# nikizadehgfdl/ocean_model_grid_generator

Measured on AMD Instinct MI355X. Metric: supergrid cells/sec (coords+metrics), 1/8° tripolar at 1/2/4/8 MI355X, higher is better.
Workload: dtype f64

## Files before the change

include/ogg_hip.h:

```cpp
#ifndef OGG_HIP_H
#define OGG_HIP_H

#ifdef __cplusplus
extern "C" {
#endif

#define OGG_OK 0
#define OGG_EORDER 1
#define OGG_ESHAPE 2
#define OGG_EHIP 3
#define OGG_ENOMEM 4
#define OGG_EARG 5

#define OGG_DP_ARC_LITERAL 0
#define OGG_DP_ARC_CHORD 1

#define OGG_SYM_DEFAULT 0
#define OGG_SYM_MIRROR 1
#define OGG_SYM_NONE 2

const char* ogg_last_error(void);
const char* ogg_version(void);
long ogg_abi_sizeof(int which);
int ogg_device_count(int* count);
// ... 177 lines not shown
    long workspace_bytes;
    int symmetry;
} ogg_dpole_band;
long ogg_dpole_band_workspace_bytes(int order, long Ni, long n_pt_rows);
int ogg_symmetry_coverage(int which, int order, long n, double lon0, double lon_dp, int symmetry, int* cell_writes, int* col_writes,
                          long* evaluated);
int ogg_supergrid_pass_dev(int n_latlon, const ogg_latlon_band* latlon, long ni1, double lon0, double lenlon, double Re, int metrics,
                           const ogg_bipolar_band* cap, const ogg_dpole_band* south_cap, void** events5, double* alg_bytes4,
                           void* stream);
int ogg_supergrid_pass_plan_dev(int n_latlon, const ogg_latlon_band* latlon, long ni1, double lon0, double lenlon, double Re, int metrics,
                                const ogg_bipolar_band* cap, const ogg_dpole_band* south_cap, void** plan_out);
int ogg_supergrid_pass_run_dev(void* plan, void** events5, double* alg_bytes4, void* stream);
int ogg_supergrid_pass_plan_destroy(void* plan);
long ogg_supergrid_pass_plan_slots(const void* plan);
long ogg_supergrid_pass_plan_carried_runs(const void* plan);
int ogg_supergrid_pass_plan_flags_dev(const void* plan, int* flags, void* stream);

int ogg_fill_dev(long n, double value, double* out, void* stream);
int ogg_bswap64_dev(long n, const void* src, void* dst, void* stream);
int ogg_libm_check_dev(int which, long n, const double* x, const double* y, unsigned long long* n_diff, void* stream);
int ogg_metrics_sums_dev(long n_dx_rows, long n_cell_rows, long ni, const double* dx, const double* dy, const double* area,
                         long col_a, long col_b, int want_first_row, int want_last_row, double* out5, void* stream);
#define OGG_QUALITY_DEGENERATE_M 1.0e-3
#define OGG_QUALITY_N_BINS 7
#define OGG_QUALITY_BIN_EDGES_DEG {1.0e-6, 1.0e-3, 0.1, 1.0, 5.0, 20.0}
enum {
    OGG_Q_DX_MIN = 0, OGG_Q_DX_MAX, OGG_Q_DY_MIN, OGG_Q_DY_MAX, OGG_Q_AREA_MIN, OGG_Q_AREA_MAX, OGG_Q_ASPECT_MAX, OGG_Q_DELTA_MAX,
    OGG_Q_RX_MAX, OGG_Q_RY_MAX, OGG_Q_RY_NEXT_MAX, OGG_Q_SEAM_MAX, OGG_Q_N_EXTREMA
};
enum {
// ... 268 lines not shown
```

ocean_model_grid_generator_amd/_lib.py:

```python
import ctypes
import os

import numpy as np

_HERE = os.path.dirname(os.path.abspath(__file__))
LIB_PATH = os.environ.get("OGG_LIB_PATH") or os.path.join(_HERE, "csrc", "libogg_hip.so")

OGG_OK, OGG_EORDER, OGG_ESHAPE, OGG_EHIP, OGG_ENOMEM, OGG_EARG = 0, 1, 2, 3, 4, 5
DP_ARC_LITERAL, DP_ARC_CHORD = 0, 1
SYM_DEFAULT, SYM_MIRROR, SYM_NONE = 0, 1, 2

c_long, c_int, c_double, c_void_p, c_longlong = ctypes.c_long, ctypes.c_int, ctypes.c_double, ctypes.c_void_p, ctypes.c_longlong
_dp = ctypes.POINTER(ctypes.c_double)
_llp = ctypes.POINTER(ctypes.c_longlong)

class LatlonBand(ctypes.Structure):
    _fields_ = [("axis_kind", c_int), ("a0", c_double), ("len", c_double), ("denom", c_double), ("y0", c_longlong),
                ("lat1d", c_void_p), ("k0", c_long), ("n_pt_rows", c_long), ("n_cell_rows", c_long), ("x", c_void_p),
                ("y", c_void_p), ("dx", c_void_p), ("dy", c_void_p), ("area", c_void_p), ("angle", c_void_p)]


class BipolarBand(ctypes.Structure):
    _fields_ = [("Ni", c_long), ("Nj", c_long), ("lat0_bp", c_double), ("lon_bp", c_double), ("rp", c_double), ("Re", c_double),
                ("order", c_int), ("symmetry", c_int), ("j0", c_long), ("n_pt_rows", c_long), ("n_cell_rows", c_long), ("x", c_void_p),
# ... 305 lines not shown
    "ogg_event_create": [ctypes.POINTER(c_void_p)],
    "ogg_event_destroy": [c_void_p],
    "ogg_event_record": [c_void_p, c_void_p],
    "ogg_event_elapsed_ms": [c_void_p, c_void_p, ctypes.POINTER(ctypes.c_float)],
    "ogg_stream_synchronize": [c_void_p],
}
STRING_GETTERS = ("ogg_last_error", "ogg_version")
LONG_GETTERS = {"ogg_abi_sizeof": [c_int],
                "ogg_bipolar_quad_workspace_bytes": [c_int, c_long, c_long],
                "ogg_displaced_pole_quad_workspace_bytes": [c_int, c_long, c_long],
                "ogg_displaced_pole_grid_workspace_bytes": [c_long, c_long],
                "ogg_dpole_band_workspace_bytes": [c_int, c_long, c_long],
                "ogg_latlon_rows_workspace_bytes": [c_int, ctypes.POINTER(LatlonBand), c_long],
                "ogg_supergrid_pass_plan_slots": [c_void_p],
                "ogg_supergrid_pass_plan_carried_runs": [c_void_p],
                "ogg_grid_quality_result_bytes": [],
                "ogg_grid_quality_workspace_bytes": [c_long, c_long],
                "ogg_topog_record_bytes": [],
                "ogg_topog_band_out_rows": [ctypes.POINTER(TopogBand)],
                "ogg_topog_workspace_bytes": [],
                "ogg_xgrid_struct_bytes": [c_int],
                "ogg_xgrid_band_first_row": [ctypes.POINTER(XgridBand)],
                "ogg_xgrid_band_out_rows": [ctypes.POINTER(XgridBand)],
                "ogg_xgrid_band_next_rows": [ctypes.POINTER(XgridBand)],
                "ogg_xgrid_workspace_bytes": [ctypes.POINTER(XgridBand), ctypes.POINTER(XgridAtm)],
                "ogg_mask_struct_bytes": [c_int],
                "ogg_mask_workspace_bytes": [ctypes.POINTER(MaskParams)],
                "ogg_remap_struct_bytes": [c_int],
                "ogg_remap_workspace_bytes": [ctypes.POINTER(RemapParams)],
                "ogg_runoff_struct_bytes": [c_int],
# ... 23 lines not shown
        try:
            import torch
        except ImportError:
            pass
    lib = ctypes.CDLL(LIB_PATH)
    for name, argtypes in SIGNATURES.items():
        if os.environ.get("OGG_LIB_PATH") and not hasattr(lib, name):
            continue
        fn = getattr(lib, name)
        fn.argtypes = argtypes
        fn.restype = c_int
    for name in STRING_GETTERS:
        getattr(lib, name).restype = ctypes.c_char_p
        getattr(lib, name).argtypes = []
    for name, argtypes in LONG_GETTERS.items():
        getattr(lib, name).restype = c_long
        getattr(lib, name).argtypes = argtypes
    _lib = lib
    return lib


def check(code):
    if code == OGG_OK:
        return
    text = load().ogg_last_error().decode("utf-8", "replace")
    if code in (OGG_EORDER, OGG_ESHAPE):
        raise Exception(text)
    raise OggHipError(code, "libogg_hip: %s" % text)


# ... 31 lines not shown
```

ocean_model_grid_generator_amd/csrc/ogg_bipolar_dev.h:

```cpp
#pragma once
#include <cstdlib>

#include "ogg_common.h"
#include "ogg_math.h"

namespace {

using namespace ogg;

struct BpRow {
    double sphig;
    double beta2_inv;
    double N_inv;
};
struct BpCol {
    double sinla;
    double alpha2;
};

OGG_DEV BpRow bp_row(double phig_in, double rp) {
    BpRow r;
    const double phig = 90 - div_pi180(2 * atan(tan(0.5 * (90 - phig_in) * kPi180) / rp));
    const double pr = phig * kPi180;
    r.sphig = sin(pr);
// ... 335 lines not shown
    m.rows_per_wg = (int)rpw;
    return dim3((unsigned)gx, (unsigned)((m.nrows + rpw - 1) / rpw));
}

constexpr double BP_GUARD_K_DEFAULT = 4000.0;

struct QuadParams {
    long nx, ny;
    double lat0_bp, lon_bp, rp, Re;
    long j0;
    long top_out_row;
    double guard_k;
    unsigned* ll_claims;
    unsigned* fix_count;
    unsigned* fix_list;
    const BpRow* row_tab;
    const BpCol* col_tab;
    double* dxq;
    double* dyq;
    double* daq;
    const double* top_src;
    QuadNodes q;
    double sx, sy, rp2p, rp2m, rp2x4, cdx, guard_kk;
};

constexpr int QS_CELLS = 63;
constexpr int QS_WAVES = 4;
constexpr int QS_WG_CELLS = QS_CELLS * QS_WAVES;

struct QuadCols {
// ... 115 lines not shown
    if (lane % M == 0 && cell < CW && c0 + cell < p.nx) p.dxq[p.top_out_row * p.nx + c0 + cell] = quad_average_1d<N>(y) * p.Re;
}

template <int N>
OGG_DEV void bipolar_tables_body(const QuadParams& p, long bx) {
    constexpr int M = N - 1;
    const long nb_tab = tables_only_blocks<N>(p);
    if (bx >= nb_tab) {
        bipolar_top_row_body<N>(p, (bx - nb_tab) * 4 + (threadIdx.x >> 6));
        return;
    }
    BpRow* row_tab = const_cast<BpRow*>(p.row_tab);
    BpCol* col_tab = const_cast<BpCol*>(p.col_tab);
    const long k = bx * blockDim.x + threadIdx.x;
    const long n_rows = M * p.ny + 2, n_cols = M * p.nx + 1;
    if (k == 0) *p.fix_count = 0u;
    for (long w = k; w < QUAD_LL_CLAIM_WORDS; w += nb_tab * blockDim.x) p.ll_claims[w] = 0u;
    if (k < n_rows) {
        double jv;
        if (k == M * p.ny)
            jv = (double)p.ny - 0.001;
        else if (k == M * p.ny + 1)
            jv = lattice_node(p.q, 0, p.ny);
        else
            jv = lattice_node(p.q, (int)(k % M), k / M);
        const double latg = p.lat0_bp + (jv * (90 - p.lat0_bp)) / (double)p.ny;
        row_tab[k] = bp_row(latg, p.rp);
    } else if (k < n_rows + n_cols) {
        const long u = k - n_rows;
        const double iv = lattice_node(p.q, (int)(u % M), u / M);
        const double lon = p.lon_bp + (iv * 360.0) / (double)p.nx;
// ... 80 lines not shown
                if (ii == 0) o.dy0 = dy;
            } else {
                const double xy = Xn * Yn;
                o.pr[ii] = (xy * rsqrt_c3(fmax(xy * (q2 * q2), tiny))) * cpr;
            }
        }
        o.guarded = 0;
        if (MODE == QM_GUARD) o.guarded = g_any | wave_next(g_first);
    }
    if (FAITHFUL) o.guarded = 0;
    if (FAITHFUL || want_dx) o.dx[M] = wave_next(o.dx[0]);
    o.pr[M] = wave_next(o.pr[0]);
}

template <int N, int MODE>
OGG_DEV void bipolar_quad_body(const QuadParams& p, const QuadRange& rg, QuadOutLds& out, long wgx, long by) {
    constexpr int M = N - 1;
    constexpr bool FAITHFUL = (MODE == QM_LITERAL);
    const int lane = threadIdx.x & 63, wave = threadIdx.x >> 6;
    const QuadLane ql = quad_lane(rg.cols, wgx, wave, lane);
    if (ql.nv == 0) return;
    const bool active = ql.active;
    const long ci = ql.ci, c0 = ql.c0;
    const int nv = ql.nv;
    const long n_cols_tab = M * p.nx + 1;
    BpCol col[M];
#pragma unroll
    for (int ii = 0; ii < M; ++ii) {
        long u = M * ci + ii;
        if (u > n_cols_tab - 1) u = n_cols_tab - 1;
        col[ii] = p.col_tab[u];
    }
    const bool cell_lane = ql.cell_lane, closing = ql.closing;
    const bool img_col = (MODE == QM_FAST) && ql.img_col;
    const long h2 = p.nx / 2;
    const QuadStores qs = quad_stores(rg.cols, ql, p.nx, MODE == QM_FAST);
// ... 49 lines not shown
                da = d * d * (Y(0, 0) + Y(0, 2) + Y(2, 0) + Y(2, 2) + 4.0 * (Y(0, 1) + Y(1, 0) + Y(1, 2) + Y(2, 1) + 4.0 * Y(1, 1)));
            } else {
                const double d = (N == 4) ? (1.0 / 12.0) : (1.0 / 180.0);
                da = d * d * ysum;
            }
            da = da * p.Re * p.Re;
        }
        const long out_r = c - p.j0;
        double* __restrict__ rdx = p.dxq + out_r * p.nx;
        double* __restrict__ rdy = p.dyq + out_r * (p.nx + 1);
        double* __restrict__ rda = p.daq + out_r * p.nx;
        if (closing) {
            rdy[ci] = dyq;
            if (img_col) rdy[h2 - ci] = dyq, rdy[h2 + ci] = dyq, rdy[p.nx - ci] = dyq;
        }
        if (cell_lane && MODE == QM_GUARD && guarded) p.fix_list[atomicAdd(p.fix_count, 1u)] = (unsigned)(out_r * p.nx + ci);
        double(*buf)[QS_WG_CELLS] = out.v[(c - r0) & 1];
        if (lane < QS_CELLS) buf[0][slot] = dxq, buf[1][slot] = dyq, buf[2][slot] = da;
        __syncthreads();
        wg_store_aligned(rdx + c0, nv, buf[0], 0, 1, wave, lane);
        wg_store_aligned(rdy + c0, nv, buf[1], 0, 1, wave, lane);
        wg_store_aligned(rda + c0, nv, buf[2], 0, 1, wave, lane);
        const int last = nv - 1;
        if (qs.n_ic > 0) {
            wg_store_aligned(rdx + qs.cell_up, qs.n_ic, buf[0], qs.k0, 1, wave, lane);
            wg_store_aligned(rda + qs.cell_up, qs.n_ic, buf[2], qs.k0, 1, wave, lane);
            wg_store_aligned(rdx + qs.cell_dn2, qs.n_ic, buf[0], last, -1, wave, lane);
            wg_store_aligned(rda + qs.cell_dn2, qs.n_ic, buf[2], last, -1, wave, lane);
            wg_store_aligned(rdx + qs.cell_dn4, qs.n_ic, buf[0], last, -1, wave, lane);
            wg_store_aligned(rda + qs.cell_dn4, qs.n_ic, buf[2], last, -1, wave, lane);
        }
        if (qs.n_ip > 0) {
            wg_store_aligned(rdy + qs.col_up, qs.n_ip, buf[1], qs.k1, 1, wave, lane);
            wg_store_aligned(rdy + qs.col_dn2, qs.n_ip, buf[1], last, -1, wave, lane);
            wg_store_aligned(rdy + qs.col_dn4, qs.n_ip, buf[1], last, -1, wave, lane);
        }
    }
}

template <int N, int MODE>
__global__ __launch_bounds__(64 * QS_WAVES) void bipolar_quad_kernel(QuadParams p, QuadRange rg) {
    __shared__ QuadOutLds out;
    bipolar_quad_body<N, MODE>(p, rg, out, blockIdx.x, blockIdx.y);
}

template <int N>
__global__ __launch_bounds__(64) void bipolar_quad_tail_kernel(QuadParams p) {
    constexpr int M = N - 1;
    __shared__ double sdx[64], sdy[64];
    const unsigned bid = blockIdx.x, nblk = gridDim.x;
    const unsigned count = *p.fix_count;
    const int lane = threadIdx.x, half = lane >> 5, q = lane & 31;
    if (p.top_src && p.top_out_row >= 0)
        for (long i = (long)bid * 64 + lane; i < p.nx; i += (long)nblk * 64) p.dxq[p.top_out_row * p.nx + i] = p.top_src[i];
    const int jj = (q < N * N) ? q / N : 0, ii = (q < N * N) ? q % N : 0;
    for (unsigned k0 = bid * 2; k0 < count; k0 += nblk * 2) {
        const unsigned k = k0 + half;
        const bool have = k < count;
        const unsigned lin = have ? p.fix_list[k] : 0u;
        const long out_r = lin / p.nx, ci = lin % p.nx;
        const long cj = p.j0 + out_r;
        double dx = 0.0, dy = 0.0;
        if (have && q < N * N) {
            const BpRow r = p.row_tab[M * cj + jj];
            const BpCol c = p.col_tab[M * ci + ii];
            double phis, rden, h_i, h_j;
            bp_point(r, c, p.rp, phis, h_i, h_j, rden);
            dx = h_i * 2 * kPi / (double)p.nx;
            dy = h_j * (90 - p.lat0_bp) * kPi180 / (double)p.ny;
        }
        __syncthreads();
        sdx[lane] = dx;
        sdy[lane] = dy;
        __syncthreads();
        if (!have || q != 0) continue;
        const int base = half << 5;
        double dxrow[N], dycol[N], dyright[N], y2[(N <= 3) ? N * N : 1];
        double ysum = 0.0;
#pragma unroll
        for (int a = 0; a < N; ++a) {
#pragma unroll
            for (int b = 0; b < N; ++b) {
                const double vx = sdx[base + a * N + b], vy = sdy[base + a * N + b];
                if (a == 0) dxrow[b] = vx;
                if (b == 0) dycol[a] = vy;
                if (b == N - 1) dyright[a] = vy;
                if (N <= 3)
                    y2[(N <= 3) ? a * N + b : 0] = vx * vy;
                else
                    ysum = ysum + (quad_weight_1d<N>(b) * quad_weight_1d<N>(a)) * (vx * vy);
            }
        }
        p.dxq[out_r * p.nx + ci] = quad_average_1d<N>(dxrow) * p.Re;
        p.dyq[out_r * (p.nx + 1) + ci] = quad_average_1d<N>(dycol) * p.Re;
        if (ci == p.nx - 1) p.dyq[out_r * (p.nx + 1) + p.nx] = quad_average_1d<N>(dyright) * p.Re;
        double da;
        if (N == 2) {
            const double d = 1.0 / 2.0;
            da = d * d * (y2[0] + y2[1] + y2[(N <= 3) ? N : 0] + y2[(N <= 3) ? N + 1 : 0]);
        } else if (N == 3) {
            const double d = 1.0 / 6.0;
            auto Y = [&](int a, int b) { return y2[(N == 3) ? a * 3 + b : 0]; };
            da = d * d * (Y(0, 0) + Y(0, 2) + Y(2, 0) + Y(2, 2) + 4.0 * (Y(0, 1) + Y(1, 0) + Y(1, 2) + Y(2, 1) + 4.0 * Y(1, 1)));
        } else {
            const double d = (N == 4) ? (1.0 / 12.0) : (1.0 / 180.0);
            da = d * d * ysum;
        }
        p.daq[out_r * p.nx + ci] = da * p.Re * p.Re;
    }
}

__global__ void bipolar_ij_kernel(long n_i, const double* __restrict__ iv, long n_j, const double* __restrict__ jv, long Ni,
                                  long Nj, double lat0_bp, double lon_bp, double rp, double* __restrict__ hi,
                                  double* __restrict__ hj) {
    const long k = (long)blockIdx.x * blockDim.x + threadIdx.x;
    const long r = blockIdx.y;
    if (k >= n_i || r >= n_j) return;
    const double lon = lon_bp + (iv[k] * 360.0) / (double)Ni;
    const double lat = lat0_bp + (jv[r] * (90 - lat0_bp)) / (double)Nj;
    const BpRow row = bp_row(lat, rp);
    const BpCol col = bp_col(lon, lon_bp);
    double phis, h_i, h_j, rden;
    bp_point(row, col, rp, phis, h_i, h_j, rden);
    hi[r * n_i + k] = h_i * 2 * kPi / (double)Ni;
// ... 60 lines not shown
    return c;
}

template <int N>
int plan_quad(QuadParams p, long n_dx_rows, long n_cell_rows, double guard_k, int symmetry, void* ws, long ws_bytes, QuadPlan& out) {
    constexpr int M = N - 1;
    const long n_rows = M * p.ny + 2, n_cols = M * p.nx + 1;
    const size_t need = quad_workspace_bytes<N>(p.nx, p.ny, n_cell_rows);
    OGG_REQUIRE(ws && (size_t)ws_bytes >= need, OGG_EARG, "bipolar quadrature workspace too small: %ld < %zu bytes", ws_bytes, need);
    BpRow* row_tab = static_cast<BpRow*>(ws);
    BpCol* col_tab = reinterpret_cast<BpCol*>(row_tab + n_rows);
    unsigned* fix_count = reinterpret_cast<unsigned*>(col_tab + n_cols);
    p.row_tab = row_tab;
    p.col_tab = col_tab;
    p.fix_count = fix_count;
    p.ll_claims = fix_count + 4;
    p.fix_list = fix_count + 4 + QUAD_LL_CLAIM_WORDS;
    p.top_src = nullptr;
    out.top_buf = reinterpret_cast<double*>(static_cast<char*>(ws) + need - (size_t)p.nx * sizeof(double));
    p.guard_k = guard_k;
    p.top_out_row = (n_dx_rows > n_cell_rows) ? n_cell_rows : -1;
    const double rp2 = p.rp * p.rp;
    p.sx = (2 * kPi) / (double)p.nx, p.sy = ((90 - p.lat0_bp) * kPi180) / (double)p.ny;
    p.rp2p = 1 + rp2, p.rp2m = 1 - rp2, p.rp2x4 = 4 * rp2;
    p.cdx = (2 * p.rp) * p.sx;
    p.guard_kk = guard_k * p.rp2x4;
    out.p = p;
    long jg = 0;
    if (guard_k > 4.0) {
        const double lat_thr = acos(2.0 / sqrt(guard_k)) / kPi180;
// ... 13 lines not shown
        long target = 4096;
        if (const char* ev = getenv("OGG_QUAD_TARGET_WAVES")) target = atol(ev) > 0 ? atol(ev) : target;
        long rpc = ((e - b) * n_strips + target - 1) / target;
        r.rows_per_chunk = rpc < 1 ? 1 : (rpc > 32 ? 32 : rpc);
        r.gy = (unsigned)((e - b + r.rows_per_chunk - 1) / r.rows_per_chunk);
        return r;
    };
    out.has_fast = lo < hi && lo < jg;
    out.has_guard = lo < hi && hi > jg;
    out.has_top = n_dx_rows > n_cell_rows;
    if (out.has_fast) out.fast = range(lo, hi < jg ? hi : jg, symmetry);
    if (out.has_guard) out.guard = range(lo > jg ? lo : jg, hi, 0);
    return OGG_OK;
}

constexpr unsigned FIXUP_BLOCKS = 2048;

template <int N>
int launch_quad_tail(const QuadPlan& q, hipStream_t s) {
    if (!q.has_guard && !(q.p.top_src && q.has_top)) return OGG_OK;
    bipolar_quad_tail_kernel<N><<<FIXUP_BLOCKS, 64, 0, s>>>(q.p);
    OGG_LAUNCH_CHECK();
    return OGG_OK;
}

template <int N>
int launch_quad(QuadParams p, long n_dx_rows, long n_cell_rows, double guard_k, int symmetry, void* ext_ws, long ext_ws_bytes, hipStream_t s) {
    const size_t need = quad_workspace_bytes<N>(p.nx, p.ny, n_cell_rows);
    void* ws = ext_ws;
    long ws_bytes = ext_ws_bytes;
    ogg::AsyncScratch own(s);
    if (!ext_ws) {
        if (int e = own.alloc(&ws, need)) return e;
        ws_bytes = (long)need;
    }
    QuadPlan q;
// ... 16 lines not shown
```

ocean_model_grid_generator_amd/csrc/ogg_pass.hip:

```cpp
#include <cstring>
#include <new>
#include <vector>

#include "ogg_bipolar_dev.h"
#include "ogg_dpole_dev.h"
#include "ogg_latlon_fused_dev.h"

extern "C" long ogg_dpole_band_workspace_bytes(int order, long Ni, long n_pt_rows);

namespace {

constexpr int PASS_TX = 256;
static_assert(PASS_TX == LF_TX && PASS_TX == 64 * MESH_WAVES && PASS_TX == 64 * QS_WAVES && PASS_TX == 64 * DM_WAVES &&
                  PASS_TX == 64 * DQ_WAVES,
              "one workgroup shape for all roles");

struct LatlonShare {
    long n_wg;
    long gx, gy;
    long strip_lo, strip_hi;
    int nt;
    unsigned* claims;
    long n_help;
    int pool;
    long points;
};

union PassLds {
    RowScalars ll[LF_ROWS + 1];
    BpRow mesh[MESH_ROWS_MAX];
    DpMeshLds dmesh;
    QuadOutLds quad;
};

struct PassAParams {
    FusedParams ll;
    LatlonShare share;
    MeshParams mesh;
    long mesh_gx, n_mesh;
    QuadParams q;
    long n_tab;
    DpQuadParams dq;
    long n_dq_tab;
    int dq_order;
    DpMeshParams dm;
    long n_dm_reset;
    long n_ll_tab;
// ... 62 lines not shown

struct PassBParams {
    FusedParams ll;
    LatlonShare share;
    MeshParams mesh;
    long mesh_gx, n_mesh;
    QuadParams q;
    QuadRange guard, fast;
    long n_guard, n_fast;
    DpMeshParams dm;
    long n_dmesh;
    DpQuadParams dq;
    long n_dquad;
    int dq_order;
    int order[5];
    const PassAParams* next;
    long n_next;
};

enum { ROLE_BP_MESH = 0, ROLE_DP_MESH, ROLE_BP_GUARD, ROLE_BP_FAST, ROLE_DP_QUAD, N_ROLES };


#ifdef OGG_TIMELINE
__device__ unsigned long long g_tl_first[8], g_tl_last_start[8], g_tl_end[8], g_tl_sum_end[8], g_tl_n[8];
__device__ unsigned long long g_tl_strip_end[512];
struct Timeline {
    unsigned long long t0;
    __device__ Timeline() : t0(wall_clock64()) {}
    __device__ void done(int r) const {
        __syncthreads();
        if (threadIdx.x == 0) {
            const unsigned long long t1 = wall_clock64();
            atomicMin(&g_tl_first[r], t0), atomicMax(&g_tl_last_start[r], t0), atomicMax(&g_tl_end[r], t1);
            atomicAdd(&g_tl_sum_end[r], t1), atomicAdd(&g_tl_n[r], 1ull);
            if (r == 0 && blockIdx.x < 512) g_tl_strip_end[blockIdx.x] = t1;
        }
    }
};
extern "C" int ogg_timeline(unsigned long long* out40, int reset) {
    unsigned long long h[40];
    const void* sym[5] = {g_tl_first, g_tl_last_start, g_tl_end, g_tl_sum_end, g_tl_n};
    for (int k = 0; k < 5; ++k)
        if (hipMemcpyFromSymbol(h + 8 * k, sym[k], 64) != hipSuccess) return 1;
    if (out40) memcpy(out40, h, sizeof h);
    if (reset) {
        unsigned long long z[8] = {}, big[8];
        for (int k = 0; k < 8; ++k) big[k] = ~0ull;
        if (hipMemcpyToSymbol(g_tl_first, big, 64) != hipSuccess) return 1;
        for (int k = 1; k < 5; ++k)
            if (hipMemcpyToSymbol(sym[k], z, 64) != hipSuccess) return 1;
    }
    return 0;
}
extern "C" int ogg_timeline_strips(unsigned long long* out512) {
    return hipMemcpyFromSymbol(out512, g_tl_strip_end, sizeof g_tl_strip_end) == hipSuccess ? 0 : 1;
}
#define OGG_TL_DONE(r) tl.done(r)
#else
#define OGG_TL_DONE(r)
#endif

template <int N, bool TAB>
__global__ __launch_bounds__(PASS_TX, TAB ? 4 : 1) void pass_b_kernel(PassBParams a) {
    __shared__ PassLds lds;
    __shared__ unsigned s_slot;
    __shared__ int s_claim;
#ifdef OGG_TIMELINE
    const Timeline tl;
#endif
    long b = blockIdx.x;
    if (b >= (long)gridDim.x - a.n_next) {
        pass_table_roles<N>(*a.next, b - ((long)gridDim.x - a.n_next));
        OGG_TL_DONE(7);
        return;
    }
    const long first_help = (long)gridDim.x - a.n_next - a.share.n_help;
    const bool helper = b >= first_help;
    if (b < a.share.n_wg || helper) {
        if (helper) {
            const long k = b - first_help, n = a.share.n_wg;
            long r = (k / 8) * 8 + (b % 8);
            b = r % n;
        }
        if (a.share.nt)
            latlon_fused_body<true, TAB>(a.ll, lds.ll, b, a.share.gx, a.share.gy, a.share.strip_lo, a.share.strip_hi, a.share.claims, helper, &s_claim, a.share.pool != 0);
        else
            latlon_fused_body<false, TAB>(a.ll, lds.ll, b, a.share.gx, a.share.gy, a.share.strip_lo, a.share.strip_hi, a.share.claims, helper, &s_claim, a.share.pool != 0);
        OGG_TL_DONE(helper ? 1 : 0);
        return;
    }
    b -= a.share.n_wg;
// ... 4 lines not shown
        const long n = (r == ROLE_BP_MESH) ? a.n_mesh : (r == ROLE_DP_MESH) ? a.n_dmesh : (r == ROLE_BP_GUARD) ? a.n_guard : (r == ROLE_BP_FAST) ? a.n_fast : a.n_dquad;
        if (role < 0) {
            if (b < n)
                role = r;
            else
                b -= n;
        }
    }
    if (role == ROLE_BP_MESH) {
        bipolar_mesh_body<false>(a.mesh, lds.mesh, b % a.mesh_gx, b / a.mesh_gx);
    } else if (role == ROLE_DP_MESH) {
        const long t = take_ticket(a.dm.ticket, &s_slot);
        dpole_mesh_body(a.dm, lds.dmesh, t % a.dm.gx, t / a.dm.gx);
    } else if (role == ROLE_BP_GUARD) {
        asm volatile("; role: guarded quadrature strips" ::: "memory");
        bipolar_quad_body<N, QM_GUARD>(a.q, a.guard, lds.quad, b % a.guard.gx, b / a.guard.gx);
    } else if (role == ROLE_BP_FAST) {
        asm volatile("; role: quadrature strips" ::: "memory");
        bipolar_quad_body<N, QM_FAST>(a.q, a.fast, lds.quad, b % a.fast.gx, b / a.fast.gx);
    } else if (role == ROLE_DP_QUAD) {
        const long strip = (b % a.dq.gx) * DQ_WAVES + (threadIdx.x >> 6), chunk = b / a.dq.gx;
        if (a.dq_order == 2)
            dpole_quad_body<2, DP_ARC_CHORD>(a.dq, strip, chunk);
        else
            dpole_quad_body<4, DP_ARC_CHORD>(a.dq, strip, chunk);
    }
    OGG_TL_DONE(2 + role);
}

template <int N>
__global__ __launch_bounds__(PASS_TX, 2) void pass_d_kernel(DpQuadParams p) {
// ... 182 lines not shown
    auto mark = [&](int k) -> int {
        if (ev && ev[k]) OGG_HIP_CHECK(hipEventRecord(ev[k], st));
        return OGG_OK;
    };
    if (alg_bytes4)
        for (int k = 0; k < 4; ++k) alg_bytes4[k] = P.alg_bytes[k];
    if (int e = mark(0)) return e;
    if (P.na > 0 && with_a) {
        pass_a_kernel<N><<<P.na, PASS_TX, 0, st>>>(P.A);
        OGG_LAUNCH_CHECK();
    }
    if (int e = mark(1)) return e;
    if (P.launch_b) {
        PassBParams b = P.B;
        if (next && n_next > 0) b.next = next, b.n_next = n_next;
        if (b.ll.row_tab)
            pass_b_kernel<N, true><<<P.nb + (unsigned)b.n_next, PASS_TX, P.b_lds_pad, st>>>(b);
        else
            pass_b_kernel<N, false><<<P.nb + (unsigned)b.n_next, PASS_TX, 0, st>>>(b);
        OGG_LAUNCH_CHECK();
    }
    if (int e = mark(2)) return e;
    if (P.have_quad) {
        if (int e = launch_quad_tail<N>(P.qp, st)) return e;
    }
    if (int e = mark(3)) return e;
    if (P.dq_literal) {
        if (P.dq_order == 2)
            pass_d_kernel<2><<<P.nd, PASS_TX, 0, st>>>(P.dq);
        else
            pass_d_kernel<4><<<P.nd, PASS_TX, 0, st>>>(P.dq);
        OGG_LAUNCH_CHECK();
    }
    return mark(4);
}

int build_pass_plan_any(int n_latlon, const ogg_latlon_band* latlon, long ni1, double lon0, double lenlon, double Re, int metrics,
                        const ogg_bipolar_band* cap, const ogg_dpole_band* south_cap, PassPlan& P, const RowScalars* row_tab = nullptr) {
// ... 80 lines not shown
            if (ran && (captured || hipStreamSynchronize(last_stream) != hipSuccess)) {
                (void)hipGetLastError();
                (void)hipDeviceSynchronize();
            }
            for (auto& slot_ws : own_ws)
                for (void* w : slot_ws)
                    if (w) (void)hipFree(w);
            for (void* w : own_row_tab)
                if (w) (void)hipFree(w);
            if (dev_a) (void)hipFree(dev_a);
            (void)hipSetDevice(current);
        }
    }
};

void route_top_row_through_workspace(PassPlan& P) {
    if (!P.have_quad || !P.qp.has_top) return;
    P.A.q.dxq = P.qp.top_buf, P.A.q.top_out_row = 0;
    P.qp.p.top_src = P.qp.top_buf;
}

int build_pass_pipe(int n_latlon, const ogg_latlon_band* latlon, long ni1, double lon0, double lenlon, double Re, int metrics,
                    const ogg_bipolar_band* cap, const ogg_dpole_band* south_cap, PassPipe& H) {
    if (int e = build_pass_plan_any(n_latlon, latlon, ni1, lon0, lenlon, Re, metrics, cap, south_cap, H.slot[0])) return e;
    if (env_long("OGG_PASS_SLOTS", 2) < 2 || !H.slot[0].launch_b || H.slot[0].na == 0) return OGG_OK;
    OGG_HIP_CHECK(hipGetDevice(&H.device));
    const bool have_cap = cap && cap->n_pt_rows > 0 && cap->workspace, have_dp = south_cap && south_cap->n_pt_rows > 0;
    H.n_slots = 2;
    const long n_tab_rows = H.slot[0].A.ll.n_bands ? H.slot[0].A.ll.row0[H.slot[0].A.ll.n_bands] : 0;
    const bool row_table = n_tab_rows > 0 && env_long("OGG_PASS_LL_TABLE", 1) != 0;
    for (int k = 0; k < 2; ++k) {
        if (row_table) {
            OGG_HIP_CHECK(hipMalloc(&H.own_row_tab[k], (size_t)n_tab_rows * sizeof(RowScalars)));
            OGG_HIP_CHECK(hipMemset(H.own_row_tab[k], 0, (size_t)n_tab_rows * sizeof(RowScalars)));
        }
        ogg_bipolar_band c{};
        ogg_dpole_band d{};
        if (have_cap) {
            c = *cap;
            OGG_HIP_CHECK(hipMalloc(&H.own_ws[k][0], (size_t)cap->workspace_bytes));
            OGG_HIP_CHECK(hipMemset(H.own_ws[k][0], 0, (size_t)cap->workspace_bytes));
            c.workspace = H.own_ws[k][0];
        }
        if (have_dp) {
            d = *south_cap;
            OGG_HIP_CHECK(hipMalloc(&H.own_ws[k][1], (size_t)south_cap->workspace_bytes));
            OGG_HIP_CHECK(hipMemset(H.own_ws[k][1], 0, (size_t)south_cap->workspace_bytes));
            d.workspace = H.own_ws[k][1];
        }
        if (int e = build_pass_plan_any(n_latlon, latlon, ni1, lon0, lenlon, Re, metrics, cap ? (have_cap ? &c : cap) : nullptr,
                                        south_cap ? (have_dp ? &d : south_cap) : nullptr, H.slot[k], static_cast<const RowScalars*>(H.own_row_tab[k])))
            return e;
    }
    for (PassPlan& P : H.slot) route_top_row_through_workspace(P);
    OGG_HIP_CHECK(hipMalloc(reinterpret_cast<void**>(&H.dev_a), 2 * sizeof(PassAParams)));
    for (int k = 0; k < 2; ++k) OGG_HIP_CHECK(hipMemcpy(H.dev_a + k, &H.slot[k].A, sizeof(PassAParams), hipMemcpyHostToDevice));
    OGG_HIP_CHECK(hipDeviceSynchronize());
    return OGG_OK;
}

int run_pass_pipe(PassPipe& H, void** events5, double* alg_bytes4, void* stream) {
    H.last_stream = ogg::as_stream(stream), H.ran = true;
    if (H.n_slots == 1) return run_pass_plan_any(H.slot[0], events5, alg_bytes4, stream);
    hipStreamCaptureStatus cap_status = hipStreamCaptureStatusNone;
    if (hipStreamIsCapturing(ogg::as_stream(stream), &cap_status) == hipSuccess && cap_status != hipStreamCaptureStatusNone) {
        const int sc = (int)(H.runs & 1ull);
        H.ready_slot = -1;
        H.captured = true;
        return run_pass_plan_any(H.slot[sc], events5, alg_bytes4, stream, true, nullptr, 0);
// ... 90 lines not shown
            }
    }
    return OGG_OK;
}

extern "C" long ogg_dpole_band_workspace_bytes(int order, long Ni, long n_pt_rows) {
    if ((order != 2 && order != 4) || Ni <= 0 || n_pt_rows < 0) return 0;
    return (long)((dm_workspace_bytes(Ni, n_pt_rows) + 255) / 256 * 256) + (long)dq_workspace_bytes(order, Ni, n_pt_rows);
}

extern "C" int ogg_supergrid_pass_dev(int n_latlon, const ogg_latlon_band* latlon, long ni1, double lon0, double lenlon, double Re, int metrics,
                                      const ogg_bipolar_band* cap, const ogg_dpole_band* south_cap, void** events5, double* alg_bytes4,
                                      void* stream) {
    PassPlan P;
    if (int e = build_pass_plan_any(n_latlon, latlon, ni1, lon0, lenlon, Re, metrics, cap, south_cap, P)) return e;
    return run_pass_plan_any(P, events5, alg_bytes4, stream);
}

extern "C" int ogg_supergrid_pass_plan_dev(int n_latlon, const ogg_latlon_band* latlon, long ni1, double lon0, double lenlon, double Re, int metrics,
                                           const ogg_bipolar_band* cap, const ogg_dpole_band* south_cap, void** plan_out) {
    OGG_REQUIRE(plan_out, OGG_EARG, "ogg_supergrid_pass_plan: null plan_out");
    *plan_out = nullptr;
    PassPipe* H = new (std::nothrow) PassPipe;
    OGG_REQUIRE(H, OGG_ENOMEM, "ogg_supergrid_pass_plan: out of host memory");
    if (int e = build_pass_pipe(n_latlon, latlon, ni1, lon0, lenlon, Re, metrics, cap, south_cap, *H)) {
        delete H;
        return e;
    }
    *plan_out = H;
    return OGG_OK;
}

extern "C" int ogg_supergrid_pass_run_dev(void* plan, void** events5, double* alg_bytes4, void* stream) {
    OGG_REQUIRE(plan, OGG_EARG, "ogg_supergrid_pass_run: null plan");
    return run_pass_pipe(*static_cast<PassPipe*>(plan), events5, alg_bytes4, stream);
}

extern "C" int ogg_supergrid_pass_plan_destroy(void* plan) {
    delete static_cast<PassPipe*>(plan);
    return OGG_OK;
}

extern "C" long ogg_supergrid_pass_plan_slots(const void* plan) { return plan ? static_cast<const PassPipe*>(plan)->n_slots : 0; }
extern "C" long ogg_supergrid_pass_plan_carried_runs(const void* plan) { return plan ? (long)static_cast<const PassPipe*>(plan)->carried_runs : 0; }

extern "C" int ogg_supergrid_pass_plan_flags_dev(const void* plan, int* flags, void* stream) {
    OGG_REQUIRE(plan && flags, OGG_EARG, "ogg_supergrid_pass_plan_flags: null pointer");
    const PassPipe& H = *static_cast<const PassPipe*>(plan);
    OGG_HIP_CHECK(hipStreamSynchronize(ogg::as_stream(stream)));
    int f = 0;
    for (int k = 0; k < H.n_slots; ++k) {
        const PassPlan& P = H.slot[k];
        unsigned w = 0u;
        if (P.B.n_dmesh > 0 && P.B.dm.ticket) {
            OGG_HIP_CHECK(hipMemcpy(&w, P.B.dm.ticket + 1, sizeof(w), hipMemcpyDeviceToHost));
            if (w) f |= 2;
        }
        if (P.dq_order && P.dq.ticket) {
            OGG_HIP_CHECK(hipMemcpy(&w, P.dq.ticket + 1, sizeof(w), hipMemcpyDeviceToHost));
            if (w) f |= 4;
        }
    }
    *flags = f;
    return OGG_OK;
}

extern "C" int ogg_tripolar_pass_events_dev(int n_latlon, const ogg_latlon_band* latlon, long ni1, double lon0, double lenlon, double Re,
                                            int metrics, const ogg_bipolar_band* cap, void** events4, double* alg_bytes3, void* stream) {
    void* ev5[5] = {nullptr, nullptr, nullptr, nullptr, nullptr};
    double by4[4] = {0.0, 0.0, 0.0, 0.0};
    if (events4)
        for (int k = 0; k < 4; ++k) ev5[k] = events4[k];
    const int rc = ogg_supergrid_pass_dev(n_latlon, latlon, ni1, lon0, lenlon, Re, metrics, cap, nullptr, events4 ? ev5 : nullptr,
                                          alg_bytes3 ? by4 : nullptr, stream);
    if (alg_bytes3)
        for (int k = 0; k < 3; ++k) alg_bytes3[k] = by4[k];
// ... 8 lines not shown
```

ocean_model_grid_generator_amd/supergrid.py:

```python
import ctypes
import math
import os

import numpy as np

from . import _lib as L
from . import ocean_grid_generator as ogg

FIELDS = ("x", "y", "dx", "dy", "area", "angle_dx")


def band(n_rows, rank, world):
    return (n_rows * rank) // world, (n_rows * (rank + 1)) // world


def band_weighted(cost, rank, world, top_capacity=1.0, capacities=None):
    c = np.concatenate(([0.0], np.cumsum(np.asarray(cost, dtype=np.float64))))
    total = c[-1]
    caps = [1.0] * (world - 1) + [float(top_capacity)] if capacities is None else [float(v) for v in capacities]
    if len(caps) != world or min(caps) <= 0.0:
        raise ValueError("band_weighted: %d capacities for %d ranks (all must be positive)" % (len(caps), world))
    before = np.concatenate(([0.0], np.cumsum(caps)))

    def edge(r):
# ... 825 lines not shown
                if s.row0 > 0:
                    e = (float("nan"), float("nan"), e[2])
                out[s.name] = e
            elif s.name == "SC":
                out[s.name] = ogg.metrics_error_from_sums(area, dy_a, dy_b, dx_first, dx_last, lat_last, lat_first, p.Re)
            else:
                out[s.name] = ogg.metrics_error_from_sums(area, dy_a, dy_b, dx_first, dx_last, lat_first, lat_last, p.Re)
        return out

    def check_lookback_flags(self):
        if self._pass_args is not None:
            flags = ctypes.c_int(0)
            L.call("ogg_supergrid_pass_plan_flags_dev", self._pass_args[4], ctypes.byref(flags), self._stream())
            if flags.value & 6:
                raise L.OggHipError(L.OGG_EHIP, "displaced-pole %s: a look-back wait timed out" % ("mesh" if flags.value & 2 else "quadrature"))
        for s in self.plan.subs:
            b = self.buf[s.name]
            if s.kind != "dpole" or b["n"] == 0:
                continue
            for off, what in ((0, "mesh"),) + (() if self.plan.skip_metrics else ((b["ws_mesh_bytes"], "quadrature"),)):
                flag = ctypes.c_int(0)
                L.call("ogg_workspace_error_flag_dev", b["ws"].data_ptr() + off, ctypes.byref(flag), self._stream())
                if flag.value != 0:
                    raise L.OggHipError(L.OGG_EHIP, "displaced-pole %s: a look-back wait timed out (flag %d)" % (what, flag.value))

    def south_cut(self):
        first = self.plan.subs[0]
        y0 = None
        if first.name == "SC" and self.plan.south_cutoff_ang > -90 and self.plan.south_cutoff_row <= 0:
            assert self.world == 1
# ... 532 lines not shown
```

Measured before the change: 121.5 billion.

## Fuse bipolar guarded-cell fix-up into pass-B kernel as a spin-waiting role

Removes the separate tail kernel launch for the bipolar quadrature fix-up by adding extra workgroups to the pass-B kernel. These workgroups wait on a guard-done counter released by the guarded strip workgroups, then recompute the flagged cells with ticket-based dynamic chunking at 256 threads. The fix-up body is also restructured: 8 cells per workgroup and the point metrics moved into a noinline helper. This saves a launch and kernel boundary, but risks spin-wait deadlock or timeout if the fix-up groups occupy slots before the guard groups are scheduled, so a timeout flag is added.

```diff
diff --git a/include/ogg_hip.h b/include/ogg_hip.h
--- a/include/ogg_hip.h
+++ b/include/ogg_hip.h
@@ -215,6 +215,7 @@
 int ogg_supergrid_pass_plan_destroy(void* plan);
 long ogg_supergrid_pass_plan_slots(const void* plan);
 long ogg_supergrid_pass_plan_carried_runs(const void* plan);
+long ogg_supergrid_pass_plan_fix_workgroups(const void* plan);
 int ogg_supergrid_pass_plan_flags_dev(const void* plan, int* flags, void* stream);
 
 int ogg_fill_dev(long n, double value, double* out, void* stream);
diff --git a/ocean_model_grid_generator_amd/_lib.py b/ocean_model_grid_generator_amd/_lib.py
--- a/ocean_model_grid_generator_amd/_lib.py
+++ b/ocean_model_grid_generator_amd/_lib.py
@@ -343,6 +343,7 @@
                 "ogg_latlon_rows_workspace_bytes": [c_int, ctypes.POINTER(LatlonBand), c_long],
                 "ogg_supergrid_pass_plan_slots": [c_void_p],
                 "ogg_supergrid_pass_plan_carried_runs": [c_void_p],
+                "ogg_supergrid_pass_plan_fix_workgroups": [c_void_p],
                 "ogg_grid_quality_result_bytes": [],
                 "ogg_grid_quality_workspace_bytes": [c_long, c_long],
                 "ogg_topog_record_bytes": [],
@@ -396,6 +397,8 @@
         getattr(lib, name).restype = ctypes.c_char_p
         getattr(lib, name).argtypes = []
     for name, argtypes in LONG_GETTERS.items():
+        if os.environ.get("OGG_LIB_PATH") and not hasattr(lib, name):
+            continue
         getattr(lib, name).restype = c_long
         getattr(lib, name).argtypes = argtypes
     _lib = lib
diff --git a/ocean_model_grid_generator_amd/csrc/ogg_bipolar_dev.h b/ocean_model_grid_generator_amd/csrc/ogg_bipolar_dev.h
--- a/ocean_model_grid_generator_amd/csrc/ogg_bipolar_dev.h
+++ b/ocean_model_grid_generator_amd/csrc/ogg_bipolar_dev.h
@@ -373,6 +373,9 @@
     unsigned* ll_claims;
     unsigned* fix_count;
     unsigned* fix_list;
+    unsigned* guard_done;
+    unsigned* fix_ticket;
+    unsigned* fix_err;
     const BpRow* row_tab;
     const BpCol* col_tab;
     double* dxq;
@@ -518,7 +521,7 @@
     BpCol* col_tab = const_cast<BpCol*>(p.col_tab);
     const long k = bx * blockDim.x + threadIdx.x;
     const long n_rows = M * p.ny + 2, n_cols = M * p.nx + 1;
-    if (k == 0) *p.fix_count = 0u;
+    if (k == 0) *p.fix_count = 0u, *p.guard_done = 0u, *p.fix_ticket = 0u;
     for (long w = k; w < QUAD_LL_CLAIM_WORDS; w += nb_tab * blockDim.x) p.ll_claims[w] = 0u;
     if (k < n_rows) {
         double jv;
@@ -629,12 +632,13 @@
 }
 
 template <int N, int MODE>
-OGG_DEV void bipolar_quad_body(const QuadParams& p, const QuadRange& rg, QuadOutLds& out, long wgx, long by) {
+OGG_DEV bool bipolar_quad_body(const QuadParams& p, const QuadRange& rg, QuadOutLds& out, long wgx, long by) {
     constexpr int M = N - 1;
     constexpr bool FAITHFUL = (MODE == QM_LITERAL);
     const int lane = threadIdx.x & 63, wave = threadIdx.x >> 6;
     const QuadLane ql = quad_lane(rg.cols, wgx, wave, lane);
-    if (ql.nv == 0) return;
+    bool handed = false;
+    if (ql.nv == 0) return handed;
     const bool active = ql.active;
     const long ci = ql.ci, c0 = ql.c0;
     const int nv = ql.nv;
@@ -714,7 +718,7 @@
             rdy[ci] = dyq;
             if (img_col) rdy[h2 - ci] = dyq, rdy[h2 + ci] = dyq, rdy[p.nx - ci] = dyq;
         }
-        if (cell_lane && MODE == QM_GUARD && guarded) p.fix_list[atomicAdd(p.fix_count, 1u)] = (unsigned)(out_r * p.nx + ci);
+        if (cell_lane && MODE == QM_GUARD && guarded) p.fix_list[atomicAdd(p.fix_count, 1u)] = (unsigned)(out_r * p.nx + ci), handed = true;
         double(*buf)[QS_WG_CELLS] = out.v[(c - r0) & 1];
         if (lane < QS_CELLS) buf[0][slot] = dxq, buf[1][slot] = dyq, buf[2][slot] = da;
         __syncthreads();
@@ -736,6 +740,7 @@
             wg_store_aligned(rdy + qs.col_dn4, qs.n_ip, buf[1], last, -1, wave, lane);
         }
     }
+    return handed;
 }
 
 template <int N, int MODE>
@@ -744,70 +749,99 @@
     bipolar_quad_body<N, MODE>(p, rg, out, blockIdx.x, blockIdx.y);
 }
 
-template <int N>
-__global__ __launch_bounds__(64) void bipolar_quad_tail_kernel(QuadParams p) {
+constexpr int FIX_TX = 256;
+constexpr int FIX_CELLS = FIX_TX / 32;
+
+struct FixLds {
+    double dx[FIX_TX], dy[FIX_TX];
+    unsigned next;
+};
+
+struct BpMetrics {
+    double h_i_inv, h_j_inv;
+};
+
+__device__ __noinline__ BpMetrics bp_point_metrics(BpRow r, BpCol c, double rp) {
+    BpMetrics m;
+    double phis, rden;
+    bp_point(r, c, rp, phis, m.h_i_inv, m.h_j_inv, rden);
+    return m;
+}
+
+template <int N>
+OGG_DEV void bipolar_fix_cells_body(const QuadParams& p, FixLds& lds, unsigned count, unsigned first, unsigned step) {
     constexpr int M = N - 1;
-    __shared__ double sdx[64], sdy[64];
-    const unsigned bid = blockIdx.x, nblk = gridDim.x;
-    const unsigned count = *p.fix_count;
-    const int lane = threadIdx.x, half = lane >> 5, q = lane & 31;
-    if (p.top_src && p.top_out_row >= 0)
-        for (long i = (long)bid * 64 + lane; i < p.nx; i += (long)nblk * 64) p.dxq[p.top_out_row * p.nx + i] = p.top_src[i];
+    const int tid = threadIdx.x, q = tid & 31, base = tid & ~31;
     const int jj = (q < N * N) ? q / N : 0, ii = (q < N * N) ? q % N : 0;
-    for (unsigned k0 = bid * 2; k0 < count; k0 += nblk * 2) {
-        const unsigned k = k0 + half;
+    const unsigned nx = (unsigned)p.nx;
+    const bool tickets = (unsigned long)step * FIX_CELLS < count;
+    unsigned chunk = first;
+    while ((unsigned long)chunk * FIX_CELLS < count) {
+        unsigned asked = ~0u;
+        if (tickets && tid == 0) asked = step + atomicAdd(p.fix_ticket, 1u);
+        const unsigned k = chunk * FIX_CELLS + (unsigned)(tid >> 5);
         const bool have = k < count;
         const unsigned lin = have ? p.fix_list[k] : 0u;
-        const long out_r = lin / p.nx, ci = lin % p.nx;
-        const long cj = p.j0 + out_r;
+        const unsigned out_r = lin / nx, ci = lin - out_r * nx;
         double dx = 0.0, dy = 0.0;
         if (have && q < N * N) {
-            const BpRow r = p.row_tab[M * cj + jj];
-            const BpCol c = p.col_tab[M * ci + ii];
-            double phis, rden, h_i, h_j;
-            bp_point(r, c, p.rp, phis, h_i, h_j, rden);
-            dx = h_i * 2 * kPi / (double)p.nx;
-            dy = h_j * (90 - p.lat0_bp) * kPi180 / (double)p.ny;
-        }
+            const BpMetrics m = bp_point_metrics(p.row_tab[M * (p.j0 + (long)out_r) + jj], p.col_tab[M * (long)ci + ii], p.rp);
+            dx = m.h_i_inv * 2 * kPi / (double)p.nx;
+            dy = m.h_j_inv * (90 - p.lat0_bp) * kPi180 / (double)p.ny;
+        }
+        lds.dx[tid] = dx, lds.dy[tid] = dy;
+        if (tid == 0) lds.next = asked;
         __syncthreads();
-        sdx[lane] = dx;
-        sdy[lane] = dy;
+        const unsigned next = lds.next;
+        if (have && q == 0) {
+            const double* vx = lds.dx + base;
+            const double* vy = lds.dy + base;
+            double dycol[N];
+#pragma unroll
+            for (int a = 0; a < N; ++a) dycol[a] = vy[a * N];
+            p.dxq[(long)out_r * p.nx + ci] = quad_average_1d<N>(vx) * p.Re;
+            p.dyq[(long)out_r * (p.nx + 1) + ci] = quad_average_1d<N>(dycol) * p.Re;
+            if (ci == nx - 1) {
+#pragma unroll
+                for (int a = 0; a < N; ++a) dycol[a] = vy[a * N + N - 1];
+                p.dyq[(long)out_r * (p.nx + 1) + p.nx] = quad_average_1d<N>(dycol) * p.Re;
+            }
+            double da;
+            if (N == 2) {
+                const double d = 1.0 / 2.0;
+                da = d * d * (vx[0] * vy[0] + vx[1] * vy[1] + vx[2] * vy[2] + vx[3] * vy[3]);
+            } else if (N == 3) {
+                const double d = 1.0 / 6.0;
+                auto Y = [&](int a, int b) { return vx[a * 3 + b] * vy[a * 3 + b]; };
+                da = d * d * (Y(0, 0) + Y(0, 2) + Y(2, 0) + Y(2, 2) + 4.0 * (Y(0, 1) + Y(1, 0) + Y(1, 2) + Y(2, 1) + 4.0 * Y(1, 1)));
+            } else {
+                double ysum = 0.0;
+#pragma unroll 1
+                for (int a = 0; a < N; ++a) {
+                    const double wa = quad_weight_1d<N>(a);
+#pragma unroll
+                    for (int b = 0; b < N; ++b) ysum = ysum + (quad_weight_1d<N>(b) * wa) * (vx[a * N + b] * vy[a * N + b]);
+                }
+                const double d = (N == 4) ? (1.0 / 12.0) : (1.0 / 180.0);
+                da = d * d * ysum;
+            }
+            p.daq[(long)out_r * p.nx + ci] = da * p.Re * p.Re;
+        }
         __syncthreads();
-        if (!have || q != 0) continue;
-        const int base = half << 5;
-        double dxrow[N], dycol[N], dyright[N], y2[(N <= 3) ? N * N : 1];
-        double ysum = 0.0;
-#pragma unroll
-        for (int a = 0; a < N; ++a) {
-#pragma unroll
-            for (int b = 0; b < N; ++b) {
-                const double vx = sdx[base + a * N + b], vy = sdy[base + a * N + b];
-                if (a == 0) dxrow[b] = vx;
-                if (b == 0) dycol[a] = vy;
-                if (b == N - 1) dyright[a] = vy;
-                if (N <= 3)
-                    y2[(N <= 3) ? a * N + b : 0] = vx * vy;
-                else
-                    ysum = ysum + (quad_weight_1d<N>(b) * quad_weight_1d<N>(a)) * (vx * vy);
-            }
-        }
-        p.dxq[out_r * p.nx + ci] = quad_average_1d<N>(dxrow) * p.Re;
-        p.dyq[out_r * (p.nx + 1) + ci] = quad_average_1d<N>(dycol) * p.Re;
-        if (ci == p.nx - 1) p.dyq[out_r * (p.nx + 1) + p.nx] = quad_average_1d<N>(dyright) * p.Re;
-        double da;
-        if (N == 2) {
-            const double d = 1.0 / 2.0;
-            da = d * d * (y2[0] + y2[1] + y2[(N <= 3) ? N : 0] + y2[(N <= 3) ? N + 1 : 0]);
-        } else if (N == 3) {
-            const double d = 1.0 / 6.0;
-            auto Y = [&](int a, int b) { return y2[(N == 3) ? a * 3 + b : 0]; };
-            da = d * d * (Y(0, 0) + Y(0, 2) + Y(2, 0) + Y(2, 2) + 4.0 * (Y(0, 1) + Y(1, 0) + Y(1, 2) + Y(2, 1) + 4.0 * Y(1, 1)));
-        } else {
-            const double d = (N == 4) ? (1.0 / 12.0) : (1.0 / 180.0);
-            da = d * d * ysum;
-        }
-        p.daq[out_r * p.nx + ci] = da * p.Re * p.Re;
-    }
+        chunk = next;
+    }
+}
+
+OGG_DEV void bipolar_copy_top_row(const QuadParams& p, unsigned w, unsigned n) {
+    if (p.top_src && p.top_out_row >= 0)
+        for (long i = (long)w * FIX_TX + threadIdx.x; i < p.nx; i += (long)n * FIX_TX) p.dxq[p.top_out_row * p.nx + i] = p.top_src[i];
+}
+
+template <int N>
+__global__ __launch_bounds__(FIX_TX) void bipolar_quad_tail_kernel(QuadParams p) {
+    __shared__ FixLds lds;
+    bipolar_copy_top_row(p, blockIdx.x, gridDim.x);
+    bipolar_fix_cells_body<N>(p, lds, *p.fix_count, blockIdx.x, gridDim.x);
 }
 
 __global__ void bipolar_ij_kernel(long n_i, const double* __restrict__ iv, long n_j, const double* __restrict__ jv, long Ni,
@@ -898,6 +932,7 @@
     p.row_tab = row_tab;
     p.col_tab = col_tab;
     p.fix_count = fix_count;
+    p.guard_done = fix_count + 1, p.fix_ticket = fix_count + 2, p.fix_err = fix_count + 3;
     p.ll_claims = fix_count + 4;
     p.fix_list = fix_count + 4 + QUAD_LL_CLAIM_WORDS;
     p.top_src = nullptr;
@@ -941,12 +976,12 @@
     return OGG_OK;
 }
 
-constexpr unsigned FIXUP_BLOCKS = 2048;
+constexpr unsigned FIXUP_BLOCKS = 512;
 
 template <int N>
 int launch_quad_tail(const QuadPlan& q, hipStream_t s) {
     if (!q.has_guard && !(q.p.top_src && q.has_top)) return OGG_OK;
-    bipolar_quad_tail_kernel<N><<<FIXUP_BLOCKS, 64, 0, s>>>(q.p);
+    bipolar_quad_tail_kernel<N><<<FIXUP_BLOCKS, FIX_TX, 0, s>>>(q.p);
     OGG_LAUNCH_CHECK();
     return OGG_OK;
 }
diff --git a/ocean_model_grid_generator_amd/csrc/ogg_pass.hip b/ocean_model_grid_generator_amd/csrc/ogg_pass.hip
--- a/ocean_model_grid_generator_amd/csrc/ogg_pass.hip
+++ b/ocean_model_grid_generator_amd/csrc/ogg_pass.hip
@@ -31,6 +31,7 @@
     BpRow mesh[MESH_ROWS_MAX];
     DpMeshLds dmesh;
     QuadOutLds quad;
+    FixLds fix;
 };
 
 struct PassAParams {
@@ -123,15 +124,37 @@
     long n_dquad;
     int dq_order;
     int order[5];
+    long n_fix;
     const PassAParams* next;
     long n_next;
 };
 
 enum { ROLE_BP_MESH = 0, ROLE_DP_MESH, ROLE_BP_GUARD, ROLE_BP_FAST, ROLE_DP_QUAD, N_ROLES };
+constexpr int ROLE_BP_FIX = N_ROLES;
+
+template <int N>
+OGG_DEV void bipolar_fix_role(const QuadParams& p, FixLds& lds, long w, long n_fix, long n_guard) {
+    bipolar_copy_top_row(p, (unsigned)w, (unsigned)n_fix);
+    if (threadIdx.x == 0) {
+        int spins = 0;
+        while (__hip_atomic_load(p.guard_done, __ATOMIC_RELAXED, __HIP_MEMORY_SCOPE_AGENT) < (unsigned)n_guard) {
+            if (++spins > LB_SPIN_LIMIT) {
+                atomicExch(p.fix_err, 1u);
+                break;
+            }
+            __builtin_amdgcn_s_sleep(8);
+        }
+        __builtin_amdgcn_fence(__ATOMIC_ACQUIRE, "agent");
+    }
+    __syncthreads();
+    const unsigned count = __hip_atomic_load(p.fix_count, __ATOMIC_RELAXED, __HIP_MEMORY_SCOPE_AGENT);
+    bipolar_fix_cells_body<N>(p, lds, count, (unsigned)w, (unsigned)n_fix);
+}
 
 
 #ifdef OGG_TIMELINE
-__device__ unsigned long long g_tl_first[8], g_tl_last_start[8], g_tl_end[8], g_tl_sum_end[8], g_tl_n[8];
+constexpr int TL_SLOTS = 9;
+__device__ unsigned long long g_tl_first[TL_SLOTS], g_tl_last_start[TL_SLOTS], g_tl_end[TL_SLOTS], g_tl_sum_end[TL_SLOTS], g_tl_n[TL_SLOTS];
 __device__ unsigned long long g_tl_strip_end[512];
 struct Timeline {
     unsigned long long t0;
@@ -146,18 +169,18 @@
         }
     }
 };
-extern "C" int ogg_timeline(unsigned long long* out40, int reset) {
-    unsigned long long h[40];
+extern "C" int ogg_timeline(unsigned long long* out45, int reset) {
+    unsigned long long h[5 * TL_SLOTS];
     const void* sym[5] = {g_tl_first, g_tl_last_start, g_tl_end, g_tl_sum_end, g_tl_n};
     for (int k = 0; k < 5; ++k)
-        if (hipMemcpyFromSymbol(h + 8 * k, sym[k], 64) != hipSuccess) return 1;
-    if (out40) memcpy(out40, h, sizeof h);
+        if (hipMemcpyFromSymbol(h + TL_SLOTS * k, sym[k], 8 * TL_SLOTS) != hipSuccess) return 1;
+    if (out45) memcpy(out45, h, sizeof h);
     if (reset) {
-        unsigned long long z[8] = {}, big[8];
-        for (int k = 0; k < 8; ++k) big[k] = ~0ull;
-        if (hipMemcpyToSymbol(g_tl_first, big, 64) != hipSuccess) return 1;
+        unsigned long long z[TL_SLOTS] = {}, big[TL_SLOTS];
+        for (int k = 0; k < TL_SLOTS; ++k) big[k] = ~0ull;
+        if (hipMemcpyToSymbol(g_tl_first, big, 8 * TL_SLOTS) != hipSuccess) return 1;
         for (int k = 1; k < 5; ++k)
-            if (hipMemcpyToSymbol(sym[k], z, 64) != hipSuccess) return 1;
+            if (hipMemcpyToSymbol(sym[k], z, 8 * TL_SLOTS) != hipSuccess) return 1;
     }
     return 0;
 }
@@ -180,10 +203,17 @@
     long b = blockIdx.x;
     if (b >= (long)gridDim.x - a.n_next) {
         pass_table_roles<N>(*a.next, b - ((long)gridDim.x - a.n_next));
-        OGG_TL_DONE(7);
-        return;
-    }
-    const long first_help = (long)gridDim.x - a.n_next - a.share.n_help;
+        OGG_TL_DONE(8);
+        return;
+    }
+    const long first_fix = (long)gridDim.x - a.n_next - a.n_fix;
+    if (b >= first_fix) {
+        asm volatile("; role: literal fix-up" ::: "memory");
+        bipolar_fix_role<N>(a.q, lds.fix, b - first_fix, a.n_fix, a.n_guard);
+        OGG_TL_DONE(2 + ROLE_BP_FIX);
+        return;
+    }
+    const long first_help = first_fix - a.share.n_help;
     const bool helper = b >= first_help;
     if (b < a.share.n_wg || helper) {
         if (helper) {
@@ -218,7 +248,17 @@
         dpole_mesh_body(a.dm, lds.dmesh, t % a.dm.gx, t / a.dm.gx);
     } else if (role == ROLE_BP_GUARD) {
         asm volatile("; role: guarded quadrature strips" ::: "memory");
-        bipolar_quad_body<N, QM_GUARD>(a.q, a.guard, lds.quad, b % a.guard.gx, b / a.guard.gx);
+        const bool handed = bipolar_quad_body<N, QM_GUARD>(a.q, a.guard, lds.quad, b % a.guard.gx, b / a.guard.gx);
+        if (a.n_fix > 0) {
+            if (threadIdx.x == 0) s_claim = 0;
+            __syncthreads();
+            if (handed) s_claim = 1;
+            __syncthreads();
+            if (threadIdx.x == 0) {
+                if (s_claim) __builtin_amdgcn_fence(__ATOMIC_RELEASE, "agent");
+                __hip_atomic_fetch_add(a.q.guard_done, 1u, __ATOMIC_RELAXED, __HIP_MEMORY_SCOPE_AGENT);
+            }
+        }
     } else if (role == ROLE_BP_FAST) {
         asm volatile("; role: quadrature strips" ::: "memory");
         bipolar_quad_body<N, QM_FAST>(a.q, a.fast, lds.quad, b % a.fast.gx, b / a.fast.gx);
@@ -431,14 +471,15 @@
     if (P.launch_b) {
         PassBParams b = P.B;
         if (next && n_next > 0) b.next = next, b.n_next = n_next;
+        const unsigned nb = P.nb + (unsigned)b.n_fix + (unsigned)b.n_next;
         if (b.ll.row_tab)
-            pass_b_kernel<N, true><<<P.nb + (unsigned)b.n_next, PASS_TX, P.b_lds_pad, st>>>(b);
+            pass_b_kernel<N, true><<<nb, PASS_TX, P.b_lds_pad, st>>>(b);
         else
-            pass_b_kernel<N, false><<<P.nb + (unsigned)b.n_next, PASS_TX, 0, st>>>(b);
+            pass_b_kernel<N, false><<<nb, PASS_TX, 0, st>>>(b);
         OGG_LAUNCH_CHECK();
     }
     if (int e = mark(2)) return e;
-    if (P.have_quad) {
+    if (P.have_quad && P.B.n_fix == 0) {
         if (int e = launch_quad_tail<N>(P.qp, st)) return e;
     }
     if (int e = mark(3)) return e;
@@ -549,6 +590,25 @@
     }
 };
 
+int fuse_fixup_into_b(PassPlan& P) {
+    const bool tail = P.have_quad && (P.qp.has_guard || (P.qp.p.top_src && P.qp.has_top));
+    const char* e = getenv("OGG_PASS_FIXUP");
+    OGG_REQUIRE(!e || !strcmp(e, "fused") || !strcmp(e, "launch"), OGG_EARG, "OGG_PASS_FIXUP=%s: fused or launch", e);
+    if (!tail || !P.launch_b || (e && !strcmp(e, "launch"))) return OGG_OK;
+    int dev = 0;
+    hipDeviceProp_t prop;
+    OGG_HIP_CHECK(hipGetDevice(&dev));
+    OGG_HIP_CHECK(hipGetDeviceProperties(&prop, dev));
+    long n = prop.multiProcessorCount;
+    const long want = env_long("OGG_PASS_FIX_WG", n);
+    if (want < n) n = want;
+    const long cells = P.qp.has_guard ? (P.qp.guard.row_end - P.qp.guard.row_begin) * P.qp.p.nx : 0;
+    if ((cells + FIX_CELLS - 1) / FIX_CELLS < n) n = (cells + FIX_CELLS - 1) / FIX_CELLS;
+    P.B.q.top_src = P.qp.p.top_src;
+    P.B.n_fix = n < 1 ? 1 : n;
+    return OGG_OK;
+}
+
 void route_top_row_through_workspace(PassPlan& P) {
     if (!P.have_quad || !P.qp.has_top) return;
     P.A.q.dxq = P.qp.top_buf, P.A.q.top_out_row = 0;
@@ -558,7 +618,7 @@
 int build_pass_pipe(int n_latlon, const ogg_latlon_band* latlon, long ni1, double lon0, double lenlon, double Re, int metrics,
                     const ogg_bipolar_band* cap, const ogg_dpole_band* south_cap, PassPipe& H) {
     if (int e = build_pass_plan_any(n_latlon, latlon, ni1, lon0, lenlon, Re, metrics, cap, south_cap, H.slot[0])) return e;
-    if (env_long("OGG_PASS_SLOTS", 2) < 2 || !H.slot[0].launch_b || H.slot[0].na == 0) return OGG_OK;
+    if (env_long("OGG_PASS_SLOTS", 2) < 2 || !H.slot[0].launch_b || H.slot[0].na == 0) return fuse_fixup_into_b(H.slot[0]);
     OGG_HIP_CHECK(hipGetDevice(&H.device));
     const bool have_cap = cap && cap->n_pt_rows > 0 && cap->workspace, have_dp = south_cap && south_cap->n_pt_rows > 0;
     H.n_slots = 2;
@@ -587,7 +647,10 @@
                                         south_cap ? (have_dp ? &d : south_cap) : nullptr, H.slot[k], static_cast<const RowScalars*>(H.own_row_tab[k])))
             return e;
     }
-    for (PassPlan& P : H.slot) route_top_row_through_workspace(P);
+    for (PassPlan& P : H.slot) {
+        route_top_row_through_workspace(P);
+        if (int e = fuse_fixup_into_b(P)) return e;
+    }
     OGG_HIP_CHECK(hipMalloc(reinterpret_cast<void**>(&H.dev_a), 2 * sizeof(PassAParams)));
     for (int k = 0; k < 2; ++k) OGG_HIP_CHECK(hipMemcpy(H.dev_a + k, &H.slot[k].A, sizeof(PassAParams), hipMemcpyHostToDevice));
     OGG_HIP_CHECK(hipDeviceSynchronize());
@@ -708,6 +771,7 @@
                                       void* stream) {
     PassPlan P;
     if (int e = build_pass_plan_any(n_latlon, latlon, ni1, lon0, lenlon, Re, metrics, cap, south_cap, P)) return e;
+    if (int e = fuse_fixup_into_b(P)) return e;
     return run_pass_plan_any(P, events5, alg_bytes4, stream);
 }
 
@@ -737,6 +801,7 @@
 
 extern "C" long ogg_supergrid_pass_plan_slots(const void* plan) { return plan ? static_cast<const PassPipe*>(plan)->n_slots : 0; }
 extern "C" long ogg_supergrid_pass_plan_carried_runs(const void* plan) { return plan ? (long)static_cast<const PassPipe*>(plan)->carried_runs : 0; }
+extern "C" long ogg_supergrid_pass_plan_fix_workgroups(const void* plan) { return plan ? static_cast<const PassPipe*>(plan)->slot[0].B.n_fix : 0; }
 
 extern "C" int ogg_supergrid_pass_plan_flags_dev(const void* plan, int* flags, void* stream) {
     OGG_REQUIRE(plan && flags, OGG_EARG, "ogg_supergrid_pass_plan_flags: null pointer");
@@ -754,6 +819,10 @@
             OGG_HIP_CHECK(hipMemcpy(&w, P.dq.ticket + 1, sizeof(w), hipMemcpyDeviceToHost));
             if (w) f |= 4;
         }
+        if (H.n_slots > 1 && P.B.n_fix > 0) {
+            OGG_HIP_CHECK(hipMemcpy(&w, P.B.q.fix_err, sizeof(w), hipMemcpyDeviceToHost));
+            if (w) f |= 8;
+        }
     }
     *flags = f;
     return OGG_OK;
diff --git a/ocean_model_grid_generator_amd/supergrid.py b/ocean_model_grid_generator_amd/supergrid.py
--- a/ocean_model_grid_generator_amd/supergrid.py
+++ b/ocean_model_grid_generator_amd/supergrid.py
@@ -863,6 +863,8 @@
             L.call("ogg_supergrid_pass_plan_flags_dev", self._pass_args[4], ctypes.byref(flags), self._stream())
             if flags.value & 6:
                 raise L.OggHipError(L.OGG_EHIP, "displaced-pole %s: a look-back wait timed out" % ("mesh" if flags.value & 2 else "quadrature"))
+            if flags.value & 8:
+                raise L.OggHipError(L.OGG_EHIP, "bipolar fix-up role: the wait for the guarded strips timed out")
         for s in self.plan.subs:
             b = self.buf[s.name]
             if s.kind != "dpole" or b["n"] == 0:
```

Result: slower. 99.87 billion (-17.8%).
